# vanTeeffelenLab/ExTrack

Measured on AMD Instinct MI355X. Metric: log-likelihood evals/sec (1e6 tracks, 2-state, len=30), higher is better.
Workload: dtype f64

## Files before the change

extrack_amd/csrc/xt_fast2.h:

```cpp
#pragma once
#include "xt_kernel.h"

#define XT_F2_CHUNK 32
#ifndef XT_F2_RENORM
#define XT_F2_RENORM 3
#endif
#define XT_F2_WAVES 4

static inline bool xt_use_fast2(int S, int NS, int F, bool preds) { return S == 2 && NS == 1 && F >= 4 && F <= 7 && !preds; }

template <int F>
struct XtF2Geom {
    static constexpr int E = 1 << F;
    static constexpr int NG = E / 2;
    static constexpr int TPW = 64 / NG;
    static constexpr int EW = E * TPW;
};

template <int F>
XT_HD int xt_f2_swz(int w)
{
    const int c4[7] = {0x5, 0x12, 0x14, 0x2c, 0x4f, 0x41, 0x15};
    const int c6[7] = {0x15, 0x36, 0x67, 0x1c, 0x2, 0x1a, 0x16};
    const int c7[7] = {0x65, 0x72, 0x6, 0x69, 0x1c, 0x4, 0x5f};
    int s = 0;
    for (int j = 0; j < 7; ++j) {
        const int col = F == 6 ? c6[j] : (F == 7 ? c7[j] : c4[j]);
        s ^= ((w >> j) & 1) ? col : 0;
    }
    return s;
}

#define XT_F2_XCLAMP XT_TCLAMP
#define XT_F2_EXP_ENTRIES 1024
#define XT_F2_EXP_BYTES (XT_F2_EXP_ENTRIES * 8)
#define XT_F2_EXP_SCALE 1477.3197218702985
#define XT_F2_EXP_HI (-6.769015308236703e-04)
#define XT_F2_EXP_LO (-1.2691901263564344e-11)
#define XT_F2_EXP_C2 0.5000000047728719
XT_HD void xt_f2_exp_bits(double t, int& j, int& e)
{
    union {
        double d;
        unsigned long long u;
    } v;
    v.d = t;
    j = (int)(v.u & (XT_F2_EXP_ENTRIES - 1));
    e = (int)(unsigned int)(v.u >> 10);
}
XT_HD void xt_exp_tab_x2(double x0, double x1, double& p0, double& p1, int& j0, int& j1, int& e0, int& e1)
{
    x0 = x0 > XT_F2_XCLAMP ? x0 : XT_F2_XCLAMP;
    x1 = x1 > XT_F2_XCLAMP ? x1 : XT_F2_XCLAMP;
    const double t0 = xt_fma(x0, XT_F2_EXP_SCALE, XT_MAGIC);
    const double t1 = xt_fma(x1, XT_F2_EXP_SCALE, XT_MAGIC);
    const double k0 = t0 - XT_MAGIC;
    const double k1 = t1 - XT_MAGIC;
    double r0 = xt_fma(k0, XT_F2_EXP_HI, x0);
    double r1 = xt_fma(k1, XT_F2_EXP_HI, x1);
    r0 = xt_fma(k0, XT_F2_EXP_LO, r0);
    r1 = xt_fma(k1, XT_F2_EXP_LO, r1);
    double q0 = 1.66666666666666666667e-01, q1 = 1.66666666666666666667e-01;
#define XT_H2(C)              \
    q0 = xt_fma(q0, r0, (C)); \
    q1 = xt_fma(q1, r1, (C));
    XT_H2(XT_F2_EXP_C2)
    XT_H2(1.0)
    XT_H2(1.0)
#undef XT_H2
    p0 = q0;
    p1 = q1;
    xt_f2_exp_bits(t0, j0, e0);
    xt_f2_exp_bits(t1, j1, e1);
}
XT_HD void xt_exp_tab_x1(double x, double& p, int& j, int& e)
{
    x = x > XT_F2_XCLAMP ? x : XT_F2_XCLAMP;
    const double t = xt_fma(x, XT_F2_EXP_SCALE, XT_MAGIC);
    const double k = t - XT_MAGIC;
    double r = xt_fma(k, XT_F2_EXP_HI, x);
    r = xt_fma(k, XT_F2_EXP_LO, r);
    double q = 1.66666666666666666667e-01;
    q = xt_fma(q, r, XT_F2_EXP_C2);
    q = xt_fma(q, r, 1.0);
    p = xt_fma(q, r, 1.0);
    xt_f2_exp_bits(t, j, e);
}
template <class Ctx>
XT_HD void xt_f2_build_exp_table(Ctx& cx, char* lds, int off, const double* T64)
{
    for (int i = cx.tid(); i < XT_F2_EXP_ENTRIES; i += cx.nthreads()) {
        const double sv = (double)(i & 15) * (XT_LN2 / 1024.0);
        double q = 1.0 / 5040.0;
        q = xt_fma(q, sv, 1.0 / 720.0);
        q = xt_fma(q, sv, 1.0 / 120.0);
        q = xt_fma(q, sv, 1.0 / 24.0);
        q = xt_fma(q, sv, 1.0 / 6.0);
        q = xt_fma(q, sv, 0.5);
        q = xt_fma(q, sv, 1.0);
        q = xt_fma(q, sv, 1.0);
        *(double*)(lds + off + i * 8) = T64[i >> 4] * q;
    }
}

template <int F, int D, int K>
struct XtF2State {
    int s01[F];
};

#define XT_F2_EXPB_OFF 1024
#define XT_F2_TAB_BYTES (1024 + XT_F2_EXP_BYTES)
#define XT_F2_T64_OFF ((XT_BLOB_HDR + XT_NTAB * 4) * 8)
#define XT_F2_NAN_OFF 832
#define XT_F2_ARR (XT_F2_WAVES * 128 * 8)
#define XT_F2_ZM0 XT_F2_TAB_BYTES
XT_HD int xt_f2_ze0(int D, int K) { return XT_F2_ZM0 + (1 + D + K) * XT_F2_ARR; }
XT_HD int xt_f2_pos0(int D, int K) { return xt_f2_ze0(D, K) + XT_F2_ARR; }
XT_HD int xt_f2_acc0(int D, int K, int KS, int tpw) { return xt_f2_pos0(D, K) + XT_F2_WAVES * tpw * XT_F2_CHUNK * (D + KS) * 8; }
XT_HD int xt_f2_block_bytes(int D, int K, int KS, int tpw) { return xt_f2_acc0(D, K, KS, tpw) + XT_F2_WAVES * 8 * 3 * 8; }

XT_HD int xt_opaque(int v)
{
#if defined(__HIP_DEVICE_COMPILE__)
    asm volatile("" : "+v"(v));
#endif
    return v;
}

template <class T>
XT_HD T& xt_at(char* lds, int byte_off)
{
#if defined(__HIP_DEVICE_COMPILE__)
    (void)lds;
    return *(__attribute__((address_space(3))) T*)(unsigned int)byte_off;
#else
    return *(T*)(lds + byte_off);
#endif
}
XT_HD void xt_f2_check_lds_base(char* lds)
{
#if defined(__HIP_DEVICE_COMPILE__)
    if ((unsigned int)(unsigned long long)(__attribute__((address_space(3))) char*)lds != 0u) __builtin_trap();
#else
    (void)lds;
#endif
}

template <int F, int D, int K, int H, bool ZF = false, bool LAZY = false>
XT_HD void xt_f2_step(char* lds, const XtF2State<F, D, K>& st, const double* c, const double* l2, const double* TT, const double* TD2)
{
    constexpr int ZEO = (1 + D + K) * XT_F2_ARR;
    const int pk = xt_opaque(st.s01[H]);
    const int a0 = pk & 0xffff, a1 = (int)((unsigned)pk >> 16);
    const double z0 = xt_at<double>(lds, a0), z1 = xt_at<double>(lds, a1);
    const int e0 = xt_at<int>(lds, a0 + ZEO), e1 = xt_at<int>(lds, a1 + ZEO);
    const int emax = e0 > e1 ? e0 : e1;
    const double w0 = xt_ldexp(z0, e0 - emax), w1 = xt_ldexp(z1, e1 - emax);
    const double W = w0 + w1;
    double M[D], U[K];
    for (int d = 0; d < D; ++d)
        M[d] = xt_fma(w1, xt_at<double>(lds, a1 + (1 + d) * XT_F2_ARR), w0 * xt_at<double>(lds, a0 + (1 + d) * XT_F2_ARR));
    for (int k = 0; k < K; ++k)
        U[k] = xt_fma(w1, xt_at<double>(lds, a1 + (1 + D + k) * XT_F2_ARR), w0 * xt_at<double>(lds, a0 + (1 + D + k) * XT_F2_ARR));
    const bool live = ZF ? true : W > 0.0;
    const double Ws = ZF ? W : (live ? W : 1.0);
    constexpr bool RN = !LAZY || (H % XT_F2_RENORM) == 0;
    const double Wm = RN ? xt_frexp_mant(W) : W;
    const int We = live ? (RN ? emax + xt_frexp_exp(W) : emax) : XT_EMIN;

    double Dq[2][K];
    for (int q = 0; q < 2; ++q)
        for (int k = 0; k < K; ++k) Dq[q][k] = xt_fma(Ws, l2[k] + TD2[q], U[k]);
    double rD[2][K], rW;
    if (K == 1) {
        const double d01 = Dq[0][0] * Dq[1][0];
        const double R = xt_rcp(Ws * d01);
        const double RW = R * Ws;
        rW = R * d01;
        rD[0][0] = RW * Dq[1][0];
        rD[1][0] = RW * Dq[0][0];
    } else {
        double f[2 * K + 1], pre[2 * K + 2], suf[2 * K + 2];
        f[0] = Ws;
        for (int q = 0; q < 2; ++q)
            for (int k = 0; k < K; ++k) f[1 + q * K + k] = Dq[q][k];
        pre[0] = 1.0;
        for (int i = 0; i < 2 * K + 1; ++i) pre[i + 1] = pre[i] * f[i];
        suf[2 * K + 1] = 1.0;
        for (int i = 2 * K; i >= 0; --i) suf[i] = suf[i + 1] * f[i];
        const double R = xt_rcp(pre[2 * K + 1]);
        rW = R * suf[1];
        for (int q = 0; q < 2; ++q)
            for (int k = 0; k < K; ++k) rD[q][k] = R * pre[1 + q * K + k] * suf[2 + q * K + k];
    }
    double dmW[D], dsqW = 0.0;
    for (int d = 0; d < D; ++d) {
        dmW[d] = xt_fma(c[d], Ws, -M[d]);
        if (K == 1) dsqW = xt_fma(dmW[d], dmW[d], dsqW);
    }
    double x[2], gf[2], tt[2][K];
    const double A = -0.5 * rW * dsqW;
    for (int q = 0; q < 2; ++q) {
        if (K == 1) {
            x[q] = A * rD[q][0];
            tt[q][0] = xt_fma(Ws, TD2[q], U[0]) * rD[q][0];
            gf[q] = xt_pow_half<D>(Ws * rD[q][0]);
        } else {
            double xx = 0.0, gg = 1.0;
            for (int d = 0; d < D; ++d) {
                xx = xt_fma(dmW[d] * dmW[d], rD[q][d], xx);
                tt[q][d] = xt_fma(Ws, TD2[q], U[d]) * rD[q][d];
                gg *= Ws * rD[q][d];
            }
            x[q] = xx * (-0.5 * rW);
            gf[q] = sqrt(gg);
        }
    }
    double p[2];
    int j[2], n[2];
    xt_exp_tab_x2(x[0], x[1], p[0], p[1], j[0], j[1], n[0], n[1]);
    for (int q = 0; q < 2; ++q) {
        const int aq = q ? a1 : a0;
        int en = We + n[q];
        const double tj = xt_at<double>(lds, XT_F2_EXPB_OFF + j[q] * 8);
        double zn = (Wm * TT[q]) * (gf[q] * tj) * p[q];
        if (!LAZY) {
            en += xt_frexp_exp(zn);
            zn = xt_frexp_mant(zn);
        }
        xt_at<double>(lds, aq) = zn;
        xt_at<int>(lds, aq + ZEO) = en > XT_EMIN ? en : XT_EMIN;
        for (int d = 0; d < D; ++d) xt_at<double>(lds, aq + (1 + d) * XT_F2_ARR) = xt_fma(dmW[d], tt[q][K == 1 ? 0 : d], M[d]) * rW;
        for (int k = 0; k < K; ++k) xt_at<double>(lds, aq + (1 + D + k) * XT_F2_ARR) = l2[k] * tt[q][k];
    }
}

// ... 233 lines not shown
```

extrack_amd/csrc/xt_math.h:

```cpp
#pragma once
#include <math.h>
#include <stdint.h>

#if defined(__HIPCC__)
#define XT_HD __host__ __device__ __forceinline__
#else
#define XT_HD inline
#endif

#if defined(__clang__)
#define XT_UNROLL _Pragma("unroll")
#else
#define XT_UNROLL
#endif

#define XT_INL __attribute__((always_inline))

#define XT_EMIN (-(1 << 30))
#define XT_LN2 0.693147180559945309417232121458
#define XT_LOG2PI 1.83787706640934548356065947281

#if defined(__HIP_DEVICE_COMPILE__)
XT_HD double xt_rcp(double x)
{
    double r = __builtin_amdgcn_rcp(x);
    double e = __builtin_fma(-x, r, 1.0);
    r = __builtin_fma(r, e, r);
    e = __builtin_fma(-x, r, 1.0);
    r = __builtin_fma(r, e, r);
    return r;
}
XT_HD double xt_frexp_mant(double x) { return __builtin_amdgcn_frexp_mant(x); }
XT_HD int xt_frexp_exp(double x) { return __builtin_amdgcn_frexp_exp(x); }
XT_HD double xt_ldexp(double x, int e) { return __builtin_amdgcn_ldexp(x, e); }
XT_HD double xt_rint(double x) { return __builtin_rint(x); }
#else
XT_HD double xt_rcp(double x) { return 1.0 / x; }
XT_HD double xt_frexp_mant(double x)
{
    int e;
    return frexp(x, &e);
}
XT_HD int xt_frexp_exp(double x)
{
    int e;
    frexp(x, &e);
    return x == 0.0 ? 0 : e;
}
XT_HD double xt_ldexp(double x, int e) { return ldexp(x, e); }
XT_HD double xt_rint(double x) { return nearbyint(x); }
#endif

XT_HD double xt_fma(double a, double b, double c) { return __builtin_fma(a, b, c); }

XT_HD double xt_rcp_fast(double x)
{
#if defined(__HIP_DEVICE_COMPILE__)
    double r = __builtin_amdgcn_rcp(x);
    const double e = __builtin_fma(-x, r, 1.0);
    return __builtin_fma(r, e, r);
#else
    return 1.0 / x;
#endif
}

XT_HD void xt_sched_fence()
{
#if defined(__HIP_DEVICE_COMPILE__)
    __builtin_amdgcn_sched_barrier(0);
#endif
}

#define XT_MAGIC 6755399441055744.0
XT_HD int xt_lo32(double t)
{
    union {
        double d;
        long long i;
    } u;
    u.d = t;
    return (int)u.i;
}

#define XT_TCLAMP (-1.1e7)
XT_HD void xt_exp_tab(double x, double& p, int& j, int& e)
{
    x = x < XT_TCLAMP ? XT_TCLAMP : x;
    const double tk = xt_fma(x, 92.33248261689366, XT_MAGIC);
    const double kf = tk - XT_MAGIC;
    double r = xt_fma(kf, -0.010830424493178725, x);
    r = xt_fma(kf, -2.030704202170295e-10, r);
    double q = 8.33333333333333333333e-03;
    q = xt_fma(q, r, 4.16666666666666666667e-02);
    q = xt_fma(q, r, 1.66666666666666666667e-01);
    q = xt_fma(q, r, 0.5);
    q = xt_fma(q, r, 1.0);
    p = xt_fma(q, r, 1.0);
    const int n = xt_lo32(tk);
    j = n & 63;
    e = n >> 6;
}

XT_HD void xt_exp_tab_fast(double x, double& p, int& j, int& e)
{
    x = x < XT_TCLAMP ? XT_TCLAMP : x;
    const double tk = xt_fma(x, 92.33248261689366, XT_MAGIC);
    const double kf = tk - XT_MAGIC;
    double r = xt_fma(kf, -0.010830424493178725, x);
    r = xt_fma(kf, -2.030704202170295e-10, r);
    double q = 4.16666666666666666667e-02;
    q = xt_fma(q, r, 1.66666666666666666667e-01);
    q = xt_fma(q, r, 0.5);
    q = xt_fma(q, r, 1.0);
    p = xt_fma(q, r, 1.0);
    const int n = xt_lo32(tk);
    j = n & 63;
    e = n >> 6;
}

template <int D>
XT_HD double xt_pow_half(double r)
{
    if (D == 1) return sqrt(r);
    if (D == 2) return r;
    if (D == 3) return r * sqrt(r);
    double o = 1.0;
    for (int d = 0; d < D / 2; ++d) o *= r;
    return (D & 1) ? o * sqrt(r) : o;
}

struct XtAcc {
    double m;
    int e;
    XT_HD void clear()
    {
        m = 0.0;
        e = XT_EMIN;
    }
    XT_HD void add(double m2, int e2)
    {
        if (m2 == 0.0) return;
        if (e2 > e) {
            m = xt_ldexp(m, e - e2) + m2;
            e = e2;
        } else {
            m += xt_ldexp(m2, e2 - e);
        }
    }
};
```

extrack_amd/csrc/xt_reg2.h:

```cpp
#pragma once
#include "xt_fast2.h"
#include "xt_grad.h"


template <int F>
struct XtR2Geom {
    static constexpr int NGB = F - 1;
    static constexpr int NG = 1 << NGB;
    static constexpr int TPW = 64 / NG;
};
XT_HD constexpr int xt_r2_gbit(int F, int i) { return F == 7 ? i : (i < 2 ? i : i + 1); }
XT_HD constexpr int xt_r2_gmask(int F) { return F == 7 ? 63 : (F == 6 ? 0x3b : (F == 5 ? 0x1b : 0x0b)); }
template <int F>
XT_HD int xt_r2_slot(int lane)
{
    if (F == 7) return 0;
    int ts = (lane >> 2) & 1;
    if (F == 5) ts |= ((lane >> 5) & 1) << 1;
    if (F == 4) ts |= ((lane >> 4) & 3) << 1;
    return ts;
}

#define XT_R2_TAN0 XT_F2_TAB_BYTES
#define XT_R2_TB 36
// ... 90 lines not shown
    }
    double dmW[D], dsqW = 0.0;
    XT_UNROLL
    for (int d = 0; d < D; ++d) {
        dmW[d] = xt_fma(c[d], Ws, -M[d]);
        if (K == 1) dsqW = xt_fma(dmW[d], dmW[d], dsqW);
    }
    double x[2], gf[2], tt[2][K];
    const double A = -0.5 * rW * dsqW;
    XT_UNROLL
    for (int q = 0; q < 2; ++q) {
        if (K == 1) {
            x[q] = A * rD[q][0];
            tt[q][0] = xt_fma(Ws, TD2[q], U[0]) * rD[q][0];
            gf[q] = xt_pow_half<D>(Ws * rD[q][0]);
        } else {
            double xx = 0.0, gg = 1.0;
            XT_UNROLL
            for (int d = 0; d < D; ++d) {
                xx = xt_fma(dmW[d] * dmW[d], rD[q][d], xx);
                tt[q][d] = xt_fma(Ws, TD2[q], U[d]) * rD[q][d];
                gg *= Ws * rD[q][d];
            }
            x[q] = xx * (-0.5 * rW);
            gf[q] = sqrt(gg);
        }
    }
    double p[2];
    int j[2], n[2];
    xt_exp_tab_x2(x[0], x[1], p[0], p[1], j[0], j[1], n[0], n[1]);
    double nz[2], nm[2][D], nu[2][K];
    int ne[2];
    XT_UNROLL
    for (int q = 0; q < 2; ++q) {
        int en = We + n[q];
        const double tj = xt_at<double>(lds, XT_F2_EXPB_OFF + j[q] * 8);
        double zn = (Wm * TT[q]) * (gf[q] * tj) * p[q];
        if (!LAZY) {
            en += xt_frexp_exp(zn);
            zn = xt_frexp_mant(zn);
        }
        nz[q] = zn;
        ne[q] = en > XT_EMIN ? en : XT_EMIN;
        XT_UNROLL
        for (int d = 0; d < D; ++d) nm[q][d] = xt_fma(dmW[d], tt[q][K == 1 ? 0 : d], M[d]) * rW;
        XT_UNROLL
        for (int k = 0; k < K; ++k) nu[q][k] = l2[k] * tt[q][k];
    }

    double a0 = 0.0, a1 = 0.0, cm[D], cu[K], dn[D], Aq[2][K], rq[2][K];
    if (NP > 0) {
        a0 = w0 * rW;
        a1 = w1 * rW;
        const double aa = a0 * a1;
        XT_UNROLL
        for (int d = 0; d < D; ++d) {
            cm[d] = aa * (s.m[0][d] - s.m[1][d]);
            dn[d] = dmW[d] * rW;
        }
        XT_UNROLL
        for (int k = 0; k < K; ++k) cu[k] = aa * (s.u[0][k] - s.u[1][k]);
        XT_UNROLL
        for (int q = 0; q < 2; ++q)
            XT_UNROLL
            for (int k = 0; k < K; ++k) {
                rq[q][k] = Ws * rD[q][k];
                if (K == 1)
                    Aq[q][0] = -0.5 * rq[q][0] * xt_fma(-(dsqW * rW * rW), rq[q][0], (double)D);
                else
                    Aq[q][k] = -0.5 * rq[q][k] * xt_fma(-(dn[k] * dn[k]), rq[q][k], 1.0);
            }
    }
    cx.template pair_exchange<XB>(nz[0], nz[1]);
    cx.template pair_exchange_i32<XB>(ne[0], ne[1]);
    XT_UNROLL
    for (int d = 0; d < D; ++d) cx.template pair_exchange<XB>(nm[0][d], nm[1][d]);
    XT_UNROLL
    for (int k = 0; k < K; ++k) cx.template pair_exchange<XB>(nu[0][k], nu[1][k]);
    XT_UNROLL
    for (int q = 0; q < 2; ++q) {
        s.z[q] = nz[q];
        s.e[q] = ne[q];
        XT_UNROLL
        for (int d = 0; d < D; ++d) s.m[q][d] = nm[q][d];
        XT_UNROLL
        for (int k = 0; k < K; ++k) s.u[q][k] = nu[q][k];
    }
    if (NP > 0) {
        XT_UNROLL
        for (int pp = 0; pp < NP; ++pp) {
            if (!(VAR & 1)) xt_sched_fence();
            const int tb = XT_R2_TAN0 + pp * XT_R2_TB * 8;
            double dl[K];
            XT_UNROLL
            for (int k = 0; k < K; ++k) dl[k] = xt_at<double>(lds, tb + k * 8);
            const double del = s.rz[pp][0] - s.rz[pp][1];
            const double R = xt_fma(a0, s.rz[pp][0], a1 * s.rz[pp][1]);
            double dmb[D], dub[K];
            XT_UNROLL
            for (int d = 0; d < D; ++d) dmb[d] = xt_fma(cm[d], del, xt_fma(a0, s.dm[pp][0][d], a1 * s.dm[pp][1][d]));
            XT_UNROLL
            for (int k = 0; k < K; ++k) dub[k] = xt_fma(cu[k], del, xt_fma(a0, s.du[pp][0][k], a1 * s.du[pp][1][k]));
            double hd[K];
            if (K == 1) {
                hd[0] = 0.0;
                XT_UNROLL
                for (int d = 0; d < D; ++d) hd[0] = xt_fma(dn[d], dmb[d], hd[0]);
            } else {
                XT_UNROLL
                for (int d = 0; d < D; ++d) hd[d] = dn[d] * dmb[d];
            }
            double trz[2], tdm[2][D], tdu[2][K];
            XT_UNROLL
            for (int q = 0; q < 2; ++q) {
                const double dlT = xt_at<double>(lds, tb + tab + io[q]);
                const double dd2 = xt_at<double>(lds, tb + XT_R2_TAB0 + 4 * 32 + io[q]);
                double rzn = R + dlT, dtt[K];
                XT_UNROLL
                for (int k = 0; k < K; ++k) {
                    const double ds2 = dd2 + dub[k], dden = dl[k] + ds2;
                    dtt[k] = rq[q][k] * xt_fma(-tt[q][k], dden, ds2);
                    rzn = xt_fma(Aq[q][k], dden, rzn);
                    rzn = xt_fma(rq[q][k], hd[k], rzn);
                    tdu[q][k] = xt_fma(l2[k], dtt[k], dl[k] * tt[q][k]);
                }
                trz[q] = ZF ? rzn : (live ? rzn : 0.0);
                XT_UNROLL
                for (int d = 0; d < D; ++d) {
                    const int kk = K == 1 ? 0 : d;
                    tdm[q][d] = xt_fma(dn[d], dtt[kk], xt_fma(-tt[q][kk], dmb[d], dmb[d]));
                }
            }
            cx.template pair_exchange<XB>(trz[0], trz[1]);
            XT_UNROLL
            for (int d = 0; d < D; ++d) cx.template pair_exchange<XB>(tdm[0][d], tdm[1][d]);
            XT_UNROLL
            for (int k = 0; k < K; ++k) cx.template pair_exchange<XB>(tdu[0][k], tdu[1][k]);
            XT_UNROLL
            for (int q = 0; q < 2; ++q) {
                s.rz[pp][q] = trz[q];
                XT_UNROLL
                for (int d = 0; d < D; ++d) s.dm[pp][q][d] = tdm[q][d];
                XT_UNROLL
                for (int k = 0; k < K; ++k) s.du[pp][q][k] = tdu[q][k];
            }
        }
    }
}

#ifndef XT_R2_RC_H
#define XT_R2_RC_H 0
#endif
#define XT_R2_RC_NONE (-2147483647 - 1)
template <int F, int D, int H, bool FIRST = false, class Ctx>
XT_HD void xt_r2_step_g(Ctx& cx, char* lds, XtR2Lane<D, 1, 0>& s, double (&lx)[2], int tab, const double* c)
{
    constexpr int NGB = F - 1;
    constexpr int XB = xt_r2_gbit(F, H), PB = xt_r2_gbit(F, (H + NGB - 1) % NGB);
    const int lane = xt_opaque(cx.lane());
    const int prev = (lane >> PB) & 1;
    const int qa = Ctx::template pair_natural<XB>() ? 0 : (lane >> XB) & 1;
    const int io[2] = {(prev * 2 + qa) * 8, (prev * 2 + (qa ^ 1)) * 8};
    double TD2[2], LT[2];
    XT_UNROLL
    for (int q = 0; q < 2; ++q) {
        TD2[q] = xt_at<double>(lds, XT_R2_TAB0 + 4 * 32 + io[q]);
        LT[q] = xt_at<double>(lds, tab + XT_R2_LNT_REL + io[q]);
    }
    const double l2 = xt_at<double>(lds, 0), nh = xt_at<double>(lds, XT_R2_GC_OFF), l22 = xt_at<double>(lds, XT_R2_GC_OFF + 8);

    double w0 = 1.0, w1 = 0.0, base = lx[0];
    if (!FIRST) {
        const double dl = lx[1] - lx[0];
        double p;
        int j, n;
        xt_exp_tab_x1(-fabs(dl), p, j, n);
        const double E = xt_ldexp(xt_at<double>(lds, XT_F2_EXPB_OFF + j * 8) * p, n);
        const bool up = dl > 0.0;
        w0 = s.z[0] * (up ? E : 1.0);
        w1 = s.z[1] * (up ? 1.0 : E);
        base = up ? lx[1] : lx[0];
    }
    const double Ws = FIRST ? 1.0 : w0 + w1;
    double M[D];
    XT_UNROLL
    for (int d = 0; d < D; ++d) M[d] = FIRST ? s.m[0][d] : xt_fma(w1, s.m[1][d], w0 * s.m[0][d]);
    const double V = FIRST ? s.u[0][0] : xt_fma(w1, s.u[1][0], w0 * s.u[0][0]);
    constexpr bool RN = !FIRST && (H % XT_F2_RENORM) == 0;
    const double Wm = FIRST ? s.z[0] : (RN ? xt_frexp_mant(Ws) : Ws);
    if (RN) base = xt_fma((double)xt_frexp_exp(Ws), XT_LN2, base);
    if (!FIRST && H == XT_R2_RC_H) {
        const int tid = xt_opaque(cx.tid());
        const int rc0 = xt_r2_rc0(D, 0, XtR2Geom<F>::TPW);
        const int cell = rc0 + (tid & ~xt_r2_gmask(F)) * 8;
        cx.atomic_max_i32(&xt_at<int>(lds, cell), (int)fmin(fmax(base, -1e9), 1e9));
        cx.wave_sync();
        const int sh = xt_at<int>(lds, cell);
        base -= (double)sh;
        xt_at<unsigned int>(lds, rc0 + XT_R2_RC_ARR + tid * 8) += (unsigned int)sh;
    }
    if (!FIRST && H == (XT_R2_RC_H + 1) % NGB) xt_at<int>(lds, xt_r2_rc0(D, 0, XtR2Geom<F>::TPW) + (xt_opaque(cx.tid()) & ~xt_r2_gmask(F)) * 8) = XT_R2_RC_NONE;

    const double Dq0 = xt_fma(Ws, TD2[0], V), Dq1 = xt_fma(Ws, TD2[1], V);
    const double d01 = Dq0 * Dq1;
    const double R = xt_rcp(Ws * d01);
    const double rW = FIRST ? 1.0 : R * d01;
    const double G = R * (Ws * (Ws * l2));
    const double g[2] = {G * Dq1, G * Dq0};
    double dn[D], dsq = 0.0;
    XT_UNROLL
    for (int d = 0; d < D; ++d) {
        dn[d] = xt_fma(c[d], Ws, -M[d]) * rW;
        dsq = xt_fma(dn[d], dn[d], dsq);
    }
    const double A = dsq * nh;
    double ny[2], nl[2], nm[2][D], nv[2];
    XT_UNROLL
    for (int q = 0; q < 2; ++q) {
        ny[q] = Wm * xt_pow_half<D>(g[q]);
        nl[q] = xt_fma(A, g[q], LT[q]) + base;
        XT_UNROLL
        for (int d = 0; d < D; ++d) nm[q][d] = xt_fma(-dn[d], g[q], c[d]);
        nv[q] = xt_fma(-l2, g[q], l22);
    }
    cx.template pair_exchange<XB>(ny[0], ny[1]);
    cx.template pair_exchange<XB>(nl[0], nl[1]);
    XT_UNROLL
    for (int d = 0; d < D; ++d) cx.template pair_exchange<XB>(nm[0][d], nm[1][d]);
    cx.template pair_exchange<XB>(nv[0], nv[1]);
    XT_UNROLL
    for (int q = 0; q < 2; ++q) {
        s.z[q] = ny[q];
        lx[q] = nl[q];
        XT_UNROLL
        for (int d = 0; d < D; ++d) s.m[q][d] = nm[q][d];
        s.u[q][0] = nv[q];
    }
}

template <int F, class Ctx>
XT_HD double xt_r2_gsum(Ctx& cx, double v)
{
    constexpr int NGB = F - 1;
    v += cx.template xor_f64<xt_r2_gbit(F, 0)>(v);
    v += cx.template xor_f64<xt_r2_gbit(F, 1)>(v);
    v += cx.template xor_f64<xt_r2_gbit(F, 2)>(v);
    if (NGB > 3) v += cx.template xor_f64<xt_r2_gbit(F, NGB > 3 ? 3 : 0)>(v);
    if (NGB > 4) v += cx.template xor_f64<xt_r2_gbit(F, NGB > 4 ? 4 : 0)>(v);
    if (NGB > 5) v += cx.template xor_f64<xt_r2_gbit(F, NGB > 5 ? 5 : 0)>(v);
    return v;
}
template <int F, class Ctx>
XT_HD int xt_r2_gmax(Ctx& cx, int v)
{
    constexpr int NGB = F - 1;
    auto mx = [](int a, int b) XT_INL { return a > b ? a : b; };
    v = mx(v, cx.template xor_i32<xt_r2_gbit(F, 0)>(v));
    v = mx(v, cx.template xor_i32<xt_r2_gbit(F, 1)>(v));
    v = mx(v, cx.template xor_i32<xt_r2_gbit(F, 2)>(v));
    if (NGB > 3) v = mx(v, cx.template xor_i32<xt_r2_gbit(F, NGB > 3 ? 3 : 0)>(v));
    if (NGB > 4) v = mx(v, cx.template xor_i32<xt_r2_gbit(F, NGB > 4 ? 4 : 0)>(v));
    if (NGB > 5) v = mx(v, cx.template xor_i32<xt_r2_gbit(F, NGB > 5 ? 5 : 0)>(v));
    return v;
}

template <int F, int D, int K, int NP, class Ctx, class GetPos>
XT_HD void xt_r2_chain(Ctx& cx, char* lds, XtR2Lane<D, K, NP>& s, int T, int stay_from, GetPos& getpos)
{
    constexpr int NGB = F - 1;
    const int lane = xt_opaque(cx.lane());
    double z = s.z[0];
    int e = s.e[0];
    XT_UNROLL
    for (int t = 1; t < NGB; ++t) {
        if (t > T) break;
        const int prev = (lane >> xt_r2_gbit(F, t == 1 ? NGB - 1 : t - 2)) & 1;
        const int q = (lane >> xt_r2_gbit(F, t - 1)) & 1;
        const int io = (prev * 2 + q) * 8;
        const double TT = xt_at<double>(lds, XT_R2_TAB0 + (t >= stay_from ? 32 : 0) + io);
        const double d2 = xt_at<double>(lds, XT_R2_TAB0 + 4 * 32 + io);
        double c[D], l2[K];
        getpos(t, c, l2);
        double tt[K], r[K], dm[D], x = 0.0, gf;
        XT_UNROLL
        for (int k = 0; k < K; ++k) {
            const double a = d2 + s.u[0][k];
            r[k] = xt_rcp(l2[k] + a);
            tt[k] = a * r[k];
        }
        XT_UNROLL
        for (int d = 0; d < D; ++d) dm[d] = c[d] - s.m[0][d];
        if (K == 1) {
            XT_UNROLL
            for (int d = 0; d < D; ++d) x = xt_fma(dm[d], dm[d], x);
            x *= -0.5 * r[0];
            gf = xt_pow_half<D>(r[0]);
        } else {
            double gg = 1.0;
            XT_UNROLL
            for (int d = 0; d < D; ++d) {
                x = xt_fma(-0.5 * dm[d] * dm[d], r[d], x);
                gg *= r[d];
            }
            gf = sqrt(gg);
        }
        double p;
        int j, n;
        xt_exp_tab_x1(x, p, j, n);
        z = (z * TT) * (gf * xt_at<double>(lds, XT_F2_EXPB_OFF + j * 8)) * p;
        e += n;
        XT_UNROLL
        for (int d = 0; d < D; ++d) s.m[0][d] = xt_fma(dm[d], tt[K == 1 ? 0 : d], s.m[0][d]);
        XT_UNROLL
        for (int k = 0; k < K; ++k) s.u[0][k] = l2[k] * tt[k];
    }
    int dummy = 0;
    XT_UNROLL
    for (int i = 0; i < NGB - 1; ++i)
        if (i >= T) dummy |= 1 << xt_r2_gbit(F, i);
    const bool live = (lane & dummy) == 0;
    s.z[0] = live ? xt_frexp_mant(z) : 0.0;
    s.e[0] = live ? e + xt_frexp_exp(z) : XT_EMIN;
}

template <int F, int D, int K, int NP, int VAR = 0, class Ctx>
XT_HD void xt_r2_body(const XtKernelArgs& a, const XtGradArgs& ga, Ctx& cx)
{
    int lb, nb;
    const XtBucketDesc b = xt_bind_bucket(a, cx.block(), cx.nblocks(), lb, nb);
    typedef XtR2Geom<F> Gm;
    constexpr int NGB = Gm::NGB, TPW = Gm::TPW;
    constexpr int GMASK = xt_r2_gmask(F);
    const int lane = cx.lane();
    const int wib = NP == 0 ? cx.uniform(cx.wave_in_block()) : cx.wave_in_block();
    const int nwb = cx.waves_per_block();
    const int L = b.L;
    const int KS = a.locerr_mode ? a.KS : 0;
    double* smem = cx.smem();
    char* lds = (char*)smem;

    const int ntab = xt_tab_doubles(2, 2);
    for (int i = cx.tid(); i < ntab; i += cx.nthreads()) smem[i] = xt_blob_ptr(a)[i];
    if (NP > 0)
        for (int i = cx.tid(); i < NP * XT_R2_TB; i += cx.nthreads()) xt_at<double>(lds, XT_R2_TAN0 + i * 8) = ga.dblob[i];
    const int NU = NP > 0 ? ga.NU : 0, NPT = NP + NU;
    for (int i = cx.tid(); i < NU * XT_R2_TB; i += cx.nthreads()) xt_at<double>(lds, XT_R2_TAN0 + (NP * XT_R2_TB + i) * 8) = ga.udblob[i];
    cx.sync();
    xt_f2_check_lds_base(lds);
    xt_f2_build_exp_table(cx, lds, XT_F2_EXPB_OFF, (const double*)(lds + XT_F2_T64_OFF));
    const bool gform = NP == 0 && K == 1 && a.well_scaled == 2 && a.locerr_mode == 0;
    if constexpr (NP == 0 && K == 1) {
        if (gform && cx.tid() < 10) {
            const int i = cx.tid();
            const double l2 = smem[0];
            if (i < 8)
                xt_at<double>(lds, XT_R2_LNT_OFF + i * 8) = log(smem[XT_BLOB_HDR + i]) - 0.5 * D * log(l2);
            else
                xt_at<double>(lds, XT_R2_GC_OFF + (i - 8) * 8) = i == 8 ? -0.5 / l2 : 2.0 * l2;
        }
    }
    cx.sync();
    const double* hdr = smem;

    const int ts = xt_r2_slot<F>(lane);
    const bool leader = (lane & GMASK) == 0;
    const int tlast = L - 1;
    const int stay_from = a.min_len > 2 ? a.min_len : 2;
    const int vfin = (b.isBL ? 2 : 0) + (tlast >= stay_from ? 1 : 0);
    double l2g[K];
    XT_UNROLL
    for (int k = 0; k < K; ++k) l2g[k] = hdr[k];
    const bool well_scaled = a.well_scaled != 0;
    const bool chain = NP == 0 && well_scaled;

    double* pos = (double*)(lds + xt_r2_pos0(NPT)) + wib * TPW * XT_F2_CHUNK * (D + KS);
    double* sig = pos + TPW * XT_F2_CHUNK * D;
    double* accp = (double*)(lds + xt_r2_acc0(NPT, D, KS, TPW)) + (wib * 8 + ts) * (NPT + 3);
    auto accb = [&]() XT_INL { return xt_r2_acc0(0, D, KS, TPW) + (wib * 8 + xt_r2_slot<F>(xt_opaque(cx.lane()))) * 24; };
    auto rcacc = [&]() XT_INL { return xt_r2_rc0(D, KS, TPW) + XT_R2_RC_ARR + xt_opaque(cx.tid()) * 8; };
    auto rcsum = [&]() XT_INL { return xt_r2_rc0(D, KS, TPW) + 2 * XT_R2_RC_ARR + (wib * 8 + xt_r2_slot<F>(xt_opaque(cx.lane()))) * 8; };
    if (leader) {
        if (NP == 0) {
            const int ab = accb();
            xt_at<double>(lds, ab) = 1.0;
            xt_at<double>(lds, ab + 8) = 0.0;
            xt_at<double>(lds, ab + 16) = 0.0;
            xt_at<double>(lds, rcsum()) = 0.0;
        } else {
            for (int i = 0; i < NPT + 1; ++i) accp[i] = 0.0;
        }
    }

    const int64_t nbatch = (b.N + TPW - 1) / TPW;
    const int64_t W0 = (int64_t)lb * nwb + wib, NW = (int64_t)nb * nwb;
    for (int64_t batch = W0; batch < nbatch; batch += NW) {
        const int64_t trk = batch * TPW + ts;
        const bool act = trk < b.N;

        auto stage = [&](int p0) XT_INL {
            cx.wave_sync();
            for (int i = lane; i < TPW * XT_F2_CHUNK * D; i += 64) {
                const int t_ = i / (XT_F2_CHUNK * D), r = i - t_ * (XT_F2_CHUNK * D);
                const int64_t tk = batch * TPW + t_;
                const int64_t tkc = tk < b.N ? tk : b.N - 1;
                const int pp = p0 + r / D;
                if (pp < L) {
                    const double v = b.tracks[(tkc * L + p0) * D + r];
                    pos[i] = v;
                    if (v != v) xt_at<int>(lds, XT_F2_NAN_OFF + (wib * 8 + t_) * 4) = 1;
                }
            }
            if (KS)
                for (int i = lane; i < TPW * XT_F2_CHUNK * KS; i += 64) {
                    const int t_ = i / (XT_F2_CHUNK * KS), r = i - t_ * (XT_F2_CHUNK * KS);
                    const int64_t tk = batch * TPW + t_;
                    const int64_t tkc = tk < b.N ? tk : b.N - 1;
                    const int pp = p0 + r / KS;
                    if (pp < L) {
                        const double v = b.sigma[(tkc * L + p0) * KS + r];
                        sig[i] = v;
                        if (v != v) xt_at<int>(lds, XT_F2_NAN_OFF + (wib * 8 + t_) * 4) = 1;
                    }
                }
            cx.wave_sync();
        };
        auto getpos = [&](int t, double* c, double* l2) XT_INL {
            const int r = t & (XT_F2_CHUNK - 1);
            XT_UNROLL
            for (int d = 0; d < D; ++d) c[d] = pos[(ts * XT_F2_CHUNK + r) * D + d];
            if (KS == 0) {
                XT_UNROLL
                for (int k = 0; k < K; ++k) l2[k] = xt_at<double>(lds, k * 8);
            } else {
                XT_UNROLL
                for (int k = 0; k < K; ++k) {
                    double sg = sig[(ts * XT_F2_CHUNK + r) * KS + (KS == 1 ? 0 : k)];
                    if (a.locerr_mode == 2) {
                        sg = xt_fma(sg, hdr[3], hdr[4]);
                        sg = sg < 1e-6 ? 1e-6 : sg;
                    }
                    l2[k] = sg * sg;
                }
            }
        };

        XtR2Lane<D, K, NP> s;
        double lx[2] = {0.0, 0.0};
#define XT_R2_PHASE(H, ZF_, LAZY_)                                                                     \
    if (NGB > (H) && t <= tend2 && ph == (H)) {                                                        \
        double c[D], l2[K];                                                                            \
        getpos(t, c, l2);                                                                              \
        xt_r2_step<F, D, K, NP, ((H) < NGB ? (H) : 0), ZF_, LAZY_, VAR>(cx, lds, s, XT_R2_TABSEL, c, l2);   \
        ++t;                                                                                           \
        ph = (H) + 1 == NGB ? 0 : (H) + 1;                                                             \
    }
#define XT_R2_PHASE_G(H)                                                                               \
    if (NGB > (H) && t <= tend2 && ph == (H)) {                                                        \
        double c[D], l2[K];                                                                            \
        getpos(t, c, l2);                                                                              \
        xt_r2_step_g<F, D, ((H) < NGB ? (H) : 0)>(cx, lds, s, lx, XT_R2_TABSEL, c);                        \
        ++t;                                                                                           \
        ph = (H) + 1 == NGB ? 0 : (H) + 1;                                                             \
    }
#define XT_R2_PHASES(ZF_, LAZY_) \
    XT_R2_PHASE(0, ZF_, LAZY_)   \
    XT_R2_PHASE(1, ZF_, LAZY_)   \
    XT_R2_PHASE(2, ZF_, LAZY_)   \
    XT_R2_PHASE(3, ZF_, LAZY_)   \
    XT_R2_PHASE(4, ZF_, LAZY_)   \
    XT_R2_PHASE(5, ZF_, LAZY_)
#define XT_R2_TABSEL tab
        auto run_steps = [&](int& t, int tend, int tab) XT_INL {
            int ph = (t - 1) % NGB;
            const int tend2 = tend;
            if (!well_scaled) {
                while (t <= tend2) { XT_R2_PHASES(false, false) }
                return;
            }
            if constexpr (NP == 0 && K == 1) {
                if (gform) {
                    while (t <= tend2) {
                        XT_R2_PHASE_G(0)
                        XT_R2_PHASE_G(1)
                        XT_R2_PHASE_G(2)
                        XT_R2_PHASE_G(3)
                        XT_R2_PHASE_G(4)
                        XT_R2_PHASE_G(5)
                    }
                    return;
                }
            }
            while (t <= tend2) { XT_R2_PHASES(true, true) }
        };
#undef XT_R2_TABSEL
#define XT_R2_TABSEL (XT_R2_TAB0 + (t >= stay_from ? 32 : 0))
        auto run_steps_g = [&](int& t, int tend) XT_INL {
            int ph = (t - 1) % NGB;
            const int tend2 = tend;
            if (well_scaled) {
                while (t <= tend2) { XT_R2_PHASES(false, true) }
            } else {
                while (t <= tend2) { XT_R2_PHASES(false, false) }
            }
        };
#undef XT_R2_TABSEL
#undef XT_R2_PHASES
#undef XT_R2_PHASE_G
#undef XT_R2_PHASE

        XtAcc tot;
        tot.clear();
        double gacc[NP ? NP : 1];
        double uacc[XT_R2_MAXU];
        int fe = XT_EMIN;
        int t = 1;
        if (lane < 8) xt_at<int>(lds, XT_F2_NAN_OFF + (wib * 8 + lane) * 4) = 0;
        if (NP == 0) {
            xt_at<int>(lds, rcacc()) = 0;
            xt_at<int>(lds, rcacc() - XT_R2_RC_ARR) = XT_R2_RC_NONE;
        }
        for (int p0 = 0; p0 < L; p0 += XT_F2_CHUNK) {
            stage(p0);
            if (p0 == 0) {
                constexpr int NBIT = xt_r2_gbit(F, NGB - 1);
                double c0[D], l20[K];
                getpos(0, c0, l20);
                const bool live0 = chain || (lane & (GMASK & ~(1 << NBIT))) == 0;
                const int s0 = (lane >> NBIT) & 1;
                s.z[0] = live0 ? hdr[8 + s0] : 0.0;
                s.e[0] = live0 ? 0 : XT_EMIN;
                s.z[1] = 0.0;
                s.e[1] = XT_EMIN;
                XT_UNROLL
                for (int q = 0; q < 2; ++q) {
                    XT_UNROLL
                    for (int d = 0; d < D; ++d) s.m[q][d] = c0[d];
                    XT_UNROLL
                    for (int k = 0; k < K; ++k) s.u[q][k] = l20[k];
                }
                XT_UNROLL
                for (int pp = 0; pp < NP; ++pp) {
                    const int tb = XT_R2_TAN0 + pp * XT_R2_TB * 8;
                    s.rz[pp][0] = live0 ? xt_at<double>(lds, tb + (8 + s0) * 8) : 0.0;
                    s.rz[pp][1] = 0.0;
                    XT_UNROLL
                    for (int q = 0; q < 2; ++q) {
                        XT_UNROLL
                        for (int d = 0; d < D; ++d) s.dm[pp][q][d] = 0.0;
                        XT_UNROLL
                        for (int k = 0; k < K; ++k) s.du[pp][q][k] = xt_at<double>(lds, tb + k * 8);
                    }
                }
                if constexpr (NP == 0) {
                    if (chain) {
                        const int T = L - 2 < NGB - 1 ? L - 2 : NGB - 1;
                        xt_r2_chain<F>(cx, lds, s, T, stay_from, getpos);
                        if (L - 2 >= F - 1) {
                            double c[D], l2[K];
                            getpos(F - 1, c, l2);
                            bool first_done = false;
                            if constexpr (K == 1) {
                                if (gform) {
                                    s.u[0][0] += l2[0];
                                    lx[0] = (double)s.e[0] * XT_LN2;
                                    xt_r2_step_g<F, D, NGB - 1, true>(cx, lds, s, lx, XT_R2_TAB0 + (F - 1 >= stay_from ? 32 : 0), c);
                                    s.e[0] = s.e[1] = 0;
                                    first_done = true;
                                }
                            }
                            if (!first_done) xt_r2_step<F, D, K, NP, NGB - 1, true, true, VAR, true>(cx, lds, s, XT_R2_TAB0 + (F - 1 >= stay_from ? 32 : 0), c, l2);
                            t = F;
                        } else {
                            t = L - 1 > 1 ? L - 1 : 1;
                        }
                    }
                }
            }
            const int tend = (L - 2 < p0 + XT_F2_CHUNK - 1) ? L - 2 : p0 + XT_F2_CHUNK - 1;
            if (NP == 0) {
                run_steps(t, tend < stay_from - 1 ? tend : stay_from - 1, XT_R2_TAB0);
                run_steps(t, tend, XT_R2_TAB0 + 32);
            } else {
                run_steps_g(t, tend);
            }
            if (tlast < p0 || tlast >= p0 + XT_F2_CHUNK) continue;
            double cl[D], l2l[K];
            getpos(tlast, cl, l2l);
            if constexpr (NP == 0 && K == 1) {
                if (gform && L - 2 >= F - 1) l2l[0] = 0.0;
            }
            const int hp = (tlast - 2 + NGB) % NGB;
            const int pbit = (F == 7 || hp < 2) ? hp : hp + 1;
            const int prev = (lane >> pbit) & 1;
            double wm[4], rr[4][K], dq[2][D], dsqQ[2];
            int we[4];
            XT_UNROLL
            for (int Q = 0; Q < 2; ++Q) {
                dsqQ[Q] = 0.0;
                XT_UNROLL
                for (int d = 0; d < D; ++d) {
                    dq[Q][d] = cl[d] - s.m[Q][d];
                    dsqQ[Q] = xt_fma(dq[Q][d], dq[Q][d], dsqQ[Q]);
                }
                double x[2], gf[2];
                XT_UNROLL
                for (int q = 0; q < 2; ++q) {
                    const double d2 = xt_at<double>(lds, XT_R2_TAB0 + 4 * 32 + (prev * 2 + q) * 8);
                    if (K == 1) {
                        const double r = xt_rcp(d2 + s.u[Q][0] + l2l[0]);
                        rr[Q * 2 + q][0] = r;
                        x[q] = -0.5 * dsqQ[Q] * r;
                        if constexpr (NP == 0) x[q] += lx[Q];
                        gf[q] = xt_pow_half<D>(r);
                    } else {
                        double xx = 0.0, gg = 1.0;
                        XT_UNROLL
                        for (int d = 0; d < D; ++d) {
                            const double r = xt_rcp(d2 + s.u[Q][d] + l2l[d]);
                            rr[Q * 2 + q][d] = r;
                            xx = xt_fma(-0.5 * dq[Q][d] * dq[Q][d], r, xx);
                            gg *= r;
                        }
                        x[q] = xx;
                        gf[q] = sqrt(gg);
                    }
                }
                double p[2];
                int j[2], n[2];
                xt_exp_tab_x2(x[0], x[1], p[0], p[1], j[0], j[1], n[0], n[1]);
                XT_UNROLL
                for (int q = 0; q < 2; ++q) {
                    const double tf = xt_at<double>(lds, XT_R2_TAB0 + vfin * 32 + (prev * 2 + q) * 8);
                    wm[Q * 2 + q] = s.z[Q] * tf * gf[q] * xt_at<double>(lds, XT_F2_EXPB_OFF + j[q] * 8) * p[q];
                    we[Q * 2 + q] = s.e[Q] + n[q];
                    tot.add(wm[Q * 2 + q], we[Q * 2 + q]);
                }
            }
            fe = xt_r2_gmax<F>(cx, tot.m != 0.0 ? tot.e : XT_EMIN);
            if (NP > 0) {
                double ws[4];
                XT_UNROLL
                for (int i = 0; i < 4; ++i) ws[i] = wm[i] != 0.0 ? xt_ldexp(wm[i], we[i] - fe) : 0.0;
                XT_UNROLL
                for (int pp = 0; pp < NP; ++pp) {
                    const int tb = XT_R2_TAN0 + pp * XT_R2_TB * 8;
                    double dl[K];
                    XT_UNROLL
                    for (int k = 0; k < K; ++k) dl[k] = xt_at<double>(lds, tb + k * 8);
                    double acc = 0.0;
                    XT_UNROLL
                    for (int Q = 0; Q < 2; ++Q) {
                        XT_UNROLL
                        for (int q = 0; q < 2; ++q) {
                            const double dlT = xt_at<double>(lds, tb + XT_R2_TAB0 + vfin * 32 + (prev * 2 + q) * 8);
                            const double dd2 = xt_at<double>(lds, tb + XT_R2_TAB0 + 4 * 32 + (prev * 2 + q) * 8);
                            double rel = s.rz[pp][Q] + dlT;
                            if (K == 1) {
                                const double r = rr[Q * 2 + q][0];
                                const double dden = dd2 + s.du[pp][Q][0] + dl[0];
                                double ddsq = 0.0;
                                XT_UNROLL
                                for (int d = 0; d < D; ++d) ddsq = xt_fma(-2.0 * dq[Q][d], s.dm[pp][Q][d], ddsq);
                                rel -= 0.5 * r * (D * dden + ddsq - dsqQ[Q] * r * dden);
                            } else {
                                XT_UNROLL
                                for (int d = 0; d < D; ++d) {
                                    const double r = rr[Q * 2 + q][d];
                                    const double dden = dd2 + s.du[pp][Q][d] + dl[d];
                                    rel -= 0.5 * r * (dden - 2.0 * dq[Q][d] * s.dm[pp][Q][d] - dq[Q][d] * dq[Q][d] * r * dden);
                                }
                            }
                            acc = xt_fma(ws[Q * 2 + q], ws[Q * 2 + q] != 0.0 ? rel : 0.0, acc);
                        }
                    }
                    gacc[pp] = acc;
                }
                XT_UNROLL
                for (int u = 0; u < XT_R2_MAXU; ++u) {
                    double acc = 0.0;
                    if (u < NU) {
                        const int tb = XT_R2_TAN0 + (NP + u) * XT_R2_TB * 8;
                        XT_UNROLL
                        for (int i = 0; i < 4; ++i) acc = xt_fma(ws[i], xt_at<double>(lds, tb + XT_R2_TAB0 + vfin * 32 + (prev * 2 + (i & 1)) * 8), acc);
                    }
                    uacc[u] = acc;
                }
            }
        }
        double sum = xt_r2_gsum<F>(cx, tot.m != 0.0 ? xt_ldexp(tot.m, tot.e - fe) : 0.0);
        const bool poisoned = xt_at<int>(lds, XT_F2_NAN_OFF + (wib * 8 + ts) * 4) != 0;
        if (poisoned) sum = NAN;
        if (NP == 0) {
            const int lz = xt_opaque(cx.lane());
            const int64_t trk = batch * TPW + xt_r2_slot<F>(lz);
            if (trk < b.N && (lz & GMASK) == 0) {
                const double rcs = (double)xt_at<int>(lds, rcacc());
                if (b.ll_out) b.ll_out[trk] = log(sum) + (double)fe * XT_LN2 + b.ll_const + rcs;
                xt_at<double>(lds, rcsum()) += rcs;
                const int ab = accb();
                const double pm = xt_at<double>(lds, ab) * xt_frexp_mant(sum);
                double acce = xt_at<double>(lds, ab + 8) + (double)(fe + xt_frexp_exp(sum) + xt_frexp_exp(pm));
                if (sum == 0.0) acce = -INFINITY;
                xt_at<double>(lds, ab) = xt_frexp_mant(pm);
                xt_at<double>(lds, ab + 8) = acce;
                xt_at<double>(lds, ab + 16) += 1.0;
            }
        } else {
            const double rs = 1.0 / sum;
            double gsum[NP ? NP : 1];
            XT_UNROLL
            for (int pp = 0; pp < NP; ++pp) gsum[pp] = xt_r2_gsum<F>(cx, gacc[pp]);
            double usum[XT_R2_MAXU];
            XT_UNROLL
            for (int u = 0; u < XT_R2_MAXU; ++u) usum[u] = u < NU ? xt_r2_gsum<F>(cx, uacc[u]) : 0.0;
            if (act && leader) {
                const double ll = log(sum) + (double)fe * XT_LN2 + b.ll_const;
                if (b.ll_out) b.ll_out[trk] = ll;
                accp[0] += ll;
                XT_UNROLL
                for (int pp = 0; pp < NP; ++pp) accp[1 + pp] += gsum[pp] * rs;
                double* const srow = b.scores_out ? b.scores_out + trk * ga.score_ld : nullptr;
                if (srow) {
                    XT_UNROLL
                    for (int pp = 0; pp < NP; ++pp) srow[ga.score_col0 + pp] = gsum[pp] * rs;
                }
                const int nsteps = L - 2 > 0 ? L - 2 : 0;
                const int n1 = nsteps >= stay_from ? nsteps - stay_from + 1 : 0, n0 = nsteps - n1;
                XT_UNROLL
                for (int u = 0; u < XT_R2_MAXU; ++u)
                    if (u < NU) {
                        const int tb = XT_R2_TAN0 + (NP + u) * XT_R2_TB * 8;
                        const double rzu = xt_at<double>(lds, tb + 8 * 8) + n0 * xt_at<double>(lds, tb + XT_R2_TAB0) + n1 * xt_at<double>(lds, tb + XT_R2_TAB0 + 32);
                        accp[1 + NP + u] += usum[u] * rs + rzu;
                        if (srow) srow[ga.score_ucol0 + u] = usum[u] * rs + rzu;
                    }
            }
        }
        cx.wave_sync();
    }

    cx.sync();
    if (NP == 0) {
        if (leader) {
            const double* ac = &xt_at<double>(lds, accb());
            smem[wib * TPW + ts] = ac[2] > 0.0 ? log(ac[0]) + ac[1] * XT_LN2 + ac[2] * b.ll_const + xt_at<double>(lds, rcsum()) : 0.0;
        }
        cx.sync();
        if (cx.tid() == 0) {
            double sacc = 0.0;
            for (int i = 0; i < nwb * TPW; ++i) sacc += smem[i];
            a.partials[cx.block()] = sacc;
        }
    } else {
        const double* acc0 = (const double*)(lds + xt_r2_acc0(NPT, D, KS, TPW));
        for (int col = cx.tid(); col < NPT + 1; col += cx.nthreads()) {
            double sacc = 0.0;
            for (int w = 0; w < nwb; ++w)
                for (int i = 0; i < TPW; ++i) sacc += acc0[(w * 8 + i) * (NPT + 3) + col];
            ga.gpartials[(int64_t)cx.block() * (NPT + 1) + col] = sacc;
        }
    }
}
```

Baseline: 432.7.

## Cut reciprocals and index math in the 2-state register step and final scoring

Restructures the per-step Gaussian update so it computes one shared reciprocal of the product of denominators and uses rescaled residuals, avoiding separate divides per branch. It adds a cheaper reciprocal refinement (one Newton step plus a quadratic correction). The final-timestep scoring now batches four reciprocals into one, the lane-dependent table offsets are precomputed once into a packed integer, and position loads use a precomputed LDS byte base. Small inline asm tweaks put a constant in a scalar register and shift tid. The aim is fewer f64 reciprocals and integer ops on the hot path, at some risk to precision and overflow from the longer product chains.

```diff
diff --git a/extrack_amd/csrc/xt_fast2.h b/extrack_amd/csrc/xt_fast2.h
--- a/extrack_amd/csrc/xt_fast2.h
+++ b/extrack_amd/csrc/xt_fast2.h
@@ -80,8 +80,12 @@
     const double k = t - XT_MAGIC;
     double r = xt_fma(k, XT_F2_EXP_HI, x);
     r = xt_fma(k, XT_F2_EXP_LO, r);
-    double q = 1.66666666666666666667e-01;
-    q = xt_fma(q, r, XT_F2_EXP_C2);
+#if defined(__HIP_DEVICE_COMPILE__)
+    double q;
+    asm("v_fma_f64 %0, %1, %2, %3" : "=v"(q) : "s"(1.66666666666666666667e-01), "v"(r), "v"(XT_F2_EXP_C2));
+#else
+    double q = xt_fma(1.66666666666666666667e-01, r, XT_F2_EXP_C2);
+#endif
     q = xt_fma(q, r, 1.0);
     p = xt_fma(q, r, 1.0);
     xt_f2_exp_bits(t, j, e);
diff --git a/extrack_amd/csrc/xt_math.h b/extrack_amd/csrc/xt_math.h
--- a/extrack_amd/csrc/xt_math.h
+++ b/extrack_amd/csrc/xt_math.h
@@ -52,6 +52,18 @@
 #endif
 
 XT_HD double xt_fma(double a, double b, double c) { return __builtin_fma(a, b, c); }
+
+XT_HD double xt_rcp3(double x)
+{
+#if defined(__HIP_DEVICE_COMPILE__)
+    double r = __builtin_amdgcn_rcp(x);
+    const double e = __builtin_fma(-x, r, 1.0);
+    const double t = __builtin_fma(e, e, e);
+    return __builtin_fma(r, t, r);
+#else
+    return 1.0 / x;
+#endif
+}
 
 XT_HD double xt_rcp_fast(double x)
 {
diff --git a/extrack_amd/csrc/xt_reg2.h b/extrack_amd/csrc/xt_reg2.h
--- a/extrack_amd/csrc/xt_reg2.h
+++ b/extrack_amd/csrc/xt_reg2.h
@@ -266,22 +266,55 @@
 #define XT_R2_RC_H 0
 #endif
 #define XT_R2_RC_NONE (-2147483647 - 1)
+#define XT_R2_IO_BITS 5
+template <int F, int H, class Ctx>
+XT_HD int xt_r2_pack_io(int lane)
+{
+    constexpr int NGB = F - 1;
+    if constexpr (H >= NGB) {
+        return 0;
+    } else {
+        constexpr int XB = xt_r2_gbit(F, H), PB = xt_r2_gbit(F, (H + NGB - 1) % NGB);
+        const int prev = (lane >> PB) & 1;
+        const int qa = Ctx::template pair_natural<XB>() ? 0 : (lane >> XB) & 1;
+        return ((prev * 2 + qa) * 8) << (XT_R2_IO_BITS * H) | xt_r2_pack_io<F, H + 1, Ctx>(lane);
+    }
+}
+XT_HD void xt_r2_opaque_inplace(int& pk)
+{
+#if defined(__HIP_DEVICE_COMPILE__)
+    asm volatile("" : "+v"(pk));
+#else
+    (void)pk;
+#endif
+}
+template <class Ctx>
+XT_HD int xt_r2_tid8(Ctx& cx)
+{
+#if defined(__HIP_DEVICE_COMPILE__)
+    int o;
+    asm volatile("v_lshlrev_b32 %0, 3, %1" : "=v"(o) : "v"(cx.tid()));
+    return o;
+#else
+    return cx.tid() * 8;
+#endif
+}
 template <int F, int D, int H, bool FIRST = false, class Ctx>
-XT_HD void xt_r2_step_g(Ctx& cx, char* lds, XtR2Lane<D, 1, 0>& s, double (&lx)[2], int tab, const double* c)
+XT_HD void xt_r2_step_g(Ctx& cx, char* lds, XtR2Lane<D, 1, 0>& s, double (&lx)[2], int& pk, int tab, const double* c)
 {
     constexpr int NGB = F - 1;
-    constexpr int XB = xt_r2_gbit(F, H), PB = xt_r2_gbit(F, (H + NGB - 1) % NGB);
-    const int lane = xt_opaque(cx.lane());
-    const int prev = (lane >> PB) & 1;
-    const int qa = Ctx::template pair_natural<XB>() ? 0 : (lane >> XB) & 1;
-    const int io[2] = {(prev * 2 + qa) * 8, (prev * 2 + (qa ^ 1)) * 8};
+    constexpr int XB = xt_r2_gbit(F, H);
+    xt_r2_opaque_inplace(pk);
+    int io0 = (int)(((unsigned int)pk >> (XT_R2_IO_BITS * H)) & ((1u << XT_R2_IO_BITS) - 1u));
+    xt_r2_opaque_inplace(io0);
+    const int io[2] = {io0, io0 ^ 8};
     double TD2[2], LT[2];
     XT_UNROLL
     for (int q = 0; q < 2; ++q) {
         TD2[q] = xt_at<double>(lds, XT_R2_TAB0 + 4 * 32 + io[q]);
         LT[q] = xt_at<double>(lds, tab + XT_R2_LNT_REL + io[q]);
     }
-    const double l2 = xt_at<double>(lds, 0), nh = xt_at<double>(lds, XT_R2_GC_OFF), l22 = xt_at<double>(lds, XT_R2_GC_OFF + 8);
+    const double l2 = xt_at<double>(lds, 0), l22 = xt_at<double>(lds, XT_R2_GC_OFF + 8);
 
     double w0 = 1.0, w1 = 0.0, base = lx[0];
     if (!FIRST) {
@@ -304,38 +337,38 @@
     const double Wm = FIRST ? s.z[0] : (RN ? xt_frexp_mant(Ws) : Ws);
     if (RN) base = xt_fma((double)xt_frexp_exp(Ws), XT_LN2, base);
     if (!FIRST && H == XT_R2_RC_H) {
-        const int tid = xt_opaque(cx.tid());
+        const int tid8 = xt_r2_tid8(cx);
         const int rc0 = xt_r2_rc0(D, 0, XtR2Geom<F>::TPW);
-        const int cell = rc0 + (tid & ~xt_r2_gmask(F)) * 8;
+        const int cell = rc0 + (tid8 & ~(xt_r2_gmask(F) * 8));
         cx.atomic_max_i32(&xt_at<int>(lds, cell), (int)fmin(fmax(base, -1e9), 1e9));
         cx.wave_sync();
         const int sh = xt_at<int>(lds, cell);
         base -= (double)sh;
-        xt_at<unsigned int>(lds, rc0 + XT_R2_RC_ARR + tid * 8) += (unsigned int)sh;
-    }
-    if (!FIRST && H == (XT_R2_RC_H + 1) % NGB) xt_at<int>(lds, xt_r2_rc0(D, 0, XtR2Geom<F>::TPW) + (xt_opaque(cx.tid()) & ~xt_r2_gmask(F)) * 8) = XT_R2_RC_NONE;
+        xt_at<unsigned int>(lds, rc0 + XT_R2_RC_ARR + tid8) += (unsigned int)sh;
+    }
+    if (!FIRST && H == (XT_R2_RC_H + 1) % NGB) xt_at<int>(lds, xt_r2_rc0(D, 0, XtR2Geom<F>::TPW) + (xt_r2_tid8(cx) & ~(xt_r2_gmask(F) * 8))) = XT_R2_RC_NONE;
 
     const double Dq0 = xt_fma(Ws, TD2[0], V), Dq1 = xt_fma(Ws, TD2[1], V);
-    const double d01 = Dq0 * Dq1;
-    const double R = xt_rcp(Ws * d01);
-    const double rW = FIRST ? 1.0 : R * d01;
-    const double G = R * (Ws * (Ws * l2));
-    const double g[2] = {G * Dq1, G * Dq0};
-    double dn[D], dsq = 0.0;
+    const double R = xt_rcp3(Ws * (Dq0 * Dq1));
+    const double h[2] = {R * Dq1, R * Dq0};
+    const double l2W = FIRST ? l2 : l2 * Ws;
+    double ed[D], esq = 0.0;
     XT_UNROLL
     for (int d = 0; d < D; ++d) {
-        dn[d] = xt_fma(c[d], Ws, -M[d]) * rW;
-        dsq = xt_fma(dn[d], dn[d], dsq);
-    }
-    const double A = dsq * nh;
+        ed[d] = FIRST ? c[d] - M[d] : xt_fma(c[d], Ws, -M[d]);
+        esq = xt_fma(ed[d], ed[d], esq);
+    }
+    const double Ah = -0.5 * esq;
+    const double WmW = FIRST ? Wm : Wm * Ws;
     double ny[2], nl[2], nm[2][D], nv[2];
     XT_UNROLL
     for (int q = 0; q < 2; ++q) {
-        ny[q] = Wm * xt_pow_half<D>(g[q]);
-        nl[q] = xt_fma(A, g[q], LT[q]) + base;
-        XT_UNROLL
-        for (int d = 0; d < D; ++d) nm[q][d] = xt_fma(-dn[d], g[q], c[d]);
-        nv[q] = xt_fma(-l2, g[q], l22);
+        const double k = l2W * h[q];
+        ny[q] = D == 2 ? WmW * k : Wm * xt_pow_half<D>(FIRST ? k : Ws * k);
+        nl[q] = xt_fma(Ah, h[q], LT[q]) + base;
+        XT_UNROLL
+        for (int d = 0; d < D; ++d) nm[q][d] = xt_fma(-ed[d], k, c[d]);
+        nv[q] = xt_fma(-l2W, k, l22);
     }
     cx.template pair_exchange<XB>(ny[0], ny[1]);
     cx.template pair_exchange<XB>(nl[0], nl[1]);
@@ -399,7 +432,7 @@
         XT_UNROLL
         for (int k = 0; k < K; ++k) {
             const double a = d2 + s.u[0][k];
-            r[k] = xt_rcp(l2[k] + a);
+            r[k] = NP == 0 ? xt_rcp3(l2[k] + a) : xt_rcp(l2[k] + a);
             tt[k] = a * r[k];
         }
         XT_UNROLL
@@ -484,11 +517,13 @@
     double l2g[K];
     XT_UNROLL
     for (int k = 0; k < K; ++k) l2g[k] = hdr[k];
+    int pk = xt_r2_pack_io<F, 0, Ctx>(lane);
     const bool well_scaled = a.well_scaled != 0;
     const bool chain = NP == 0 && well_scaled;
 
     double* pos = (double*)(lds + xt_r2_pos0(NPT)) + wib * TPW * XT_F2_CHUNK * (D + KS);
     double* sig = pos + TPW * XT_F2_CHUNK * D;
+    const int posb = NP == 0 ? xt_opaque(xt_r2_pos0(0) + (wib * TPW * XT_F2_CHUNK * (D + KS) + ts * XT_F2_CHUNK * D) * 8) : 0;
     double* accp = (double*)(lds + xt_r2_acc0(NPT, D, KS, TPW)) + (wib * 8 + ts) * (NPT + 3);
     auto accb = [&]() XT_INL { return xt_r2_acc0(0, D, KS, TPW) + (wib * 8 + xt_r2_slot<F>(xt_opaque(cx.lane()))) * 24; };
     auto rcacc = [&]() XT_INL { return xt_r2_rc0(D, KS, TPW) + XT_R2_RC_ARR + xt_opaque(cx.tid()) * 8; };
@@ -541,7 +576,7 @@
         auto getpos = [&](int t, double* c, double* l2) XT_INL {
             const int r = t & (XT_F2_CHUNK - 1);
             XT_UNROLL
-            for (int d = 0; d < D; ++d) c[d] = pos[(ts * XT_F2_CHUNK + r) * D + d];
+            for (int d = 0; d < D; ++d) c[d] = NP == 0 ? xt_at<double>(lds, posb + (r * D + d) * 8) : pos[(ts * XT_F2_CHUNK + r) * D + d];
             if (KS == 0) {
                 XT_UNROLL
                 for (int k = 0; k < K; ++k) l2[k] = xt_at<double>(lds, k * 8);
@@ -572,7 +607,7 @@
     if (NGB > (H) && t <= tend2 && ph == (H)) {                                                        \
         double c[D], l2[K];                                                                            \
         getpos(t, c, l2);                                                                              \
-        xt_r2_step_g<F, D, ((H) < NGB ? (H) : 0)>(cx, lds, s, lx, XT_R2_TABSEL, c);                        \
+        xt_r2_step_g<F, D, ((H) < NGB ? (H) : 0)>(cx, lds, s, lx, pk, XT_R2_TABSEL, c);                    \
         ++t;                                                                                           \
         ph = (H) + 1 == NGB ? 0 : (H) + 1;                                                             \
     }
@@ -677,7 +712,7 @@
                                 if (gform) {
                                     s.u[0][0] += l2[0];
                                     lx[0] = (double)s.e[0] * XT_LN2;
-                                    xt_r2_step_g<F, D, NGB - 1, true>(cx, lds, s, lx, XT_R2_TAB0 + (F - 1 >= stay_from ? 32 : 0), c);
+                                    xt_r2_step_g<F, D, NGB - 1, true>(cx, lds, s, lx, pk, XT_R2_TAB0 + (F - 1 >= stay_from ? 32 : 0), c);
                                     s.e[0] = s.e[1] = 0;
                                     first_done = true;
                                 }
@@ -708,6 +743,18 @@
             const int prev = (lane >> pbit) & 1;
             double wm[4], rr[4][K], dq[2][D], dsqQ[2];
             int we[4];
+            if constexpr (NP == 0 && K == 1) {
+                double dn[4];
+                XT_UNROLL
+                for (int i = 0; i < 4; ++i) dn[i] = xt_at<double>(lds, XT_R2_TAB0 + 4 * 32 + (prev * 2 + (i & 1)) * 8) + s.u[i >> 1][0] + l2l[0];
+                const double p01 = dn[0] * dn[1], p23 = dn[2] * dn[3];
+                const double R = xt_rcp3(p01 * p23);
+                const double r01 = R * p23, r23 = R * p01;
+                rr[0][0] = r01 * dn[1];
+                rr[1][0] = r01 * dn[0];
+                rr[2][0] = r23 * dn[3];
+                rr[3][0] = r23 * dn[2];
+            }
             XT_UNROLL
             for (int Q = 0; Q < 2; ++Q) {
                 dsqQ[Q] = 0.0;
@@ -721,8 +768,13 @@
                 for (int q = 0; q < 2; ++q) {
                     const double d2 = xt_at<double>(lds, XT_R2_TAB0 + 4 * 32 + (prev * 2 + q) * 8);
                     if (K == 1) {
-                        const double r = xt_rcp(d2 + s.u[Q][0] + l2l[0]);
-                        rr[Q * 2 + q][0] = r;
+                        double r;
+                        if constexpr (NP == 0) {
+                            r = rr[Q * 2 + q][0];
+                        } else {
+                            r = xt_rcp(d2 + s.u[Q][0] + l2l[0]);
+                            rr[Q * 2 + q][0] = r;
+                        }
                         x[q] = -0.5 * dsqQ[Q] * r;
                         if constexpr (NP == 0) x[q] += lx[Q];
                         gf[q] = xt_pow_half<D>(r);
@@ -730,7 +782,7 @@
                         double xx = 0.0, gg = 1.0;
                         XT_UNROLL
                         for (int d = 0; d < D; ++d) {
-                            const double r = xt_rcp(d2 + s.u[Q][d] + l2l[d]);
+                            const double r = NP == 0 ? xt_rcp3(d2 + s.u[Q][d] + l2l[d]) : xt_rcp(d2 + s.u[Q][d] + l2l[d]);
                             rr[Q * 2 + q][d] = r;
                             xx = xt_fma(-0.5 * dq[Q][d] * dq[Q][d], r, xx);
                             gg *= r;
```

Result: faster. 464.3, median of 6 (+7.3%).
